# kokkos/kokkos-kernels

Measured on AMD Instinct MI355X. Metric: SpMV GFLOP/s (CSR, 27-pt 3-D FE Laplacian, fp64), higher is better.
Workload: dtype f64

## Files before the change

### kokkos-kernels_amd/csrc/kk_spmv_mv4.h

```cpp
#pragma once
#include "kk_spmv_plan.h"
#include <climits>

namespace kk {

constexpr int kMv4Threads = 512, kMv4RI = 32, kMv4RJ = 4, kMv4MaxL = 28;
__host__ __device__ constexpr int mv4_pitch(int ne, int vbytes) {
  return ((ne * vbytes) % 128 == 0) ? ne + 2 * (8 / vbytes) : ne;
}

struct Mv4Tab { int n; int e[kMv4MaxL]; };
constexpr int kMv4MaxG = 9;
struct Mv4Groups {
  int n, ng;
  int e[kMv4MaxG];
  int pres[kMv4MaxG];
  int perm[kMv4MaxL];
  int ent[kMv4MaxL];
};

}

struct kkamd_mv4_plan {
  int nx = 0, ny = 0, nz = 0, kc = 0, kc1 = 0, kc1_planes = 0;
  int64_t S1 = 0, S2 = 0, npi = 0, npj = 0, nchunk = 0, nchunk1 = 0, n_nc = 0;
  kk::Mv4Groups grp{};
  void* d_arow = nullptr;
  uint32_t* d_amask = nullptr;
  int32_t* d_nc = nullptr;
  size_t bytes = 0;
};

namespace kk {

template <class OffT, class AT>
__global__ __launch_bounds__(kBlock) void mv4_rows_kernel(int64_t n_list, const int32_t* __restrict__ list, const OffT* __restrict__ row_map,
                                                          const int32_t* __restrict__ entries, const AT* __restrict__ values,
                                                          const double* __restrict__ X, int64_t xs0, int64_t xs1, double* __restrict__ Y,
                                                          int64_t ys0, int64_t ys1, double alpha, double beta, int ncv) {
  int64_t idx = ((int64_t)blockIdx.x * kBlock + threadIdx.x) / 16;
  const int j  = threadIdx.x & 15;
  const int jc = j < ncv ? j : ncv - 1;
  const bool live = idx < n_list;
  if (!live) idx = n_list - 1;
  const int64_t r = list[idx];
  const int64_t b = (int64_t)row_map[r], e = (int64_t)row_map[r + 1];
  double acc = 0.0;
  for (int64_t a = b; a < e; a += 16) {
    const bool in = a + j < e;
    const int32_t my_col = in ? entries[a + j] : 0;
    const double my_val  = in ? (double)values[a + j] : 0.0;
    KK_UNROLL
    for (int q = 0; q < 16; ++q) {
      const int32_t col = __shfl(my_col, q, 16);
      const double v    = __shfl(my_val, q, 16);
      const double x    = X[(int64_t)col * xs0 + jc * xs1];
      acc = (a + q < e) ? acc + v * x : acc;
    }
  }
  if (!live || j >= ncv) return;
  double* yp = Y + r * ys0 + j * ys1;
  *yp = (beta == 0.0) ? alpha * acc : beta * (*yp) + alpha * acc;
}

template <class OffT, class AT, int NG, unsigned PRES, bool BETA0, int XM, bool PART = false>
__global__ __launch_bounds__(kMv4Threads, 1) void spmv_mv4_kernel(const OffT* __restrict__ arow, const uint32_t* __restrict__ amask, const AT* __restrict__ values, Mv4Groups G,
                                                                  const double* __restrict__ X0, int64_t xs0, int64_t xs1, double* __restrict__ Y0,
                                                                  int64_t ys0, int64_t ys1, double alpha, double beta, int y_vec_ok, int nx,
                                                                  int ny, int nz, int64_t S1, int64_t S2, int64_t npi, int64_t npj, int kc, int ncv_last, int ncb) {
  constexpr bool XROW = XM == 1;
  constexpr bool XT   = XM == 2;
  constexpr int RI = kMv4RI, RJ = kMv4RJ, W = RI + 2, SLABR = (RJ + 2) * W, SLABB = SLABR * 128, NT = kMv4Threads;
  constexpr int ROWS = NT / 8;
  constexpr int NP = SLABR * 8, NXP = (NP + NT - 1) / NT;
  constexpr int NPOS = 3 * NG + (NG & 1);
  constexpr int LP = mv4_pitch(NPOS, (int)sizeof(AT));
  constexpr int AV = (3 * NG + 7) / 8;
  using XV = kk_f64x2;
  using AV2 = typename vec2<AT>::type;
  KK_DYN_SMEM(char, smem);
  __shared__ int perm_s[kMv4MaxL];
  char* ring = smem;
  AT* abuf   = reinterpret_cast<AT*>(smem + 4 * (size_t)SLABB);
  const int t = threadIdx.x, rs = t >> 3, line = rs / RI, ii = rs % RI, c = t & 7;
  const int64_t bb = xcd_remap(blockIdx.x, gridDim.x);
  const int64_t b = ncb > 1 ? bb / ncb : bb;
  const int64_t cblk = ncb > 1 ? bb - b * ncb : 0;
  const double* __restrict__ X = X0 + cblk * 16 * xs1;
  double* __restrict__ Y = Y0 + cblk * 16 * ys1;
  const int ncv = (PART && cblk != ncb - 1) ? 16 : ncv_last;
  const int64_t npatch = npi * npj;
  const int64_t ch = b / npatch, p = b % npatch;
  const int i0 = (int)(p % npi) * RI, j0 = (int)(p / npi) * RJ;
  const int kbeg = (int)ch * kc, kend = (kbeg + kc < nz) ? kbeg + kc : nz;
  const int njj = (j0 + RJ <= ny) ? RJ : ny - j0;
  bool lane_ok[2];
  const OffT* wbase[2]; const uint32_t* mbase[2]; double* ybase[2];
  KK_UNROLL
  for (int u = 0; u < 2; ++u) {
    const int jj = 2 * line + u;
    lane_ok[u] = jj < njj && i0 + ii < nx;
    const int64_t r0 = lane_ok[u] ? (int64_t)(j0 + jj) * S1 + i0 + ii : 0;
    wbase[u] = arow + r0; mbase[u] = amask + r0;
    ybase[u] = Y + r0 * ys0 + (2 * c) * ys1;
  }
  const bool ycol0 = !PART || 2 * c < ncv, ycol1 = !PART || 2 * c + 1 < ncv;
  const double* xbase[NXP];
  unsigned xsec_none = 0;
  bool x_in[NXP];
  int x_dst[XT ? NXP : 1];
  unsigned x_live = 0;
  KK_UNROLL
  for (int it = 0; it < NXP; ++it) {
    int g = it * NT + t;
    int xr, part;
    if constexpr (!XT) { g = g < NP ? g : NP - 1; xr = g >> 3; part = g & 7; }
    else {
      part = g / SLABR; xr = g - part * SLABR;
      if (part > 7) { part = 7; xr = SLABR; }
      if (xr < SLABR) x_live |= 1u << it; else xr = SLABR - 1;
      x_dst[it] = (xr * 8 + (part ^ ((xr % W) & 7))) * 16;
    }
    const int jr = j0 - 1 + xr / W, ir = i0 - 1 + xr % W;
    x_in[it] = jr >= 0 && jr < ny && ir >= 0 && ir < nx;
    const int jq = jr < 0 ? 0 : (jr > ny - 1 ? ny - 1 : jr), iq = ir < 0 ? 0 : (ir > nx - 1 ? nx - 1 : ir);
    const int col0 = !PART ? 2 * part : (XROW ? (2 * part + 1 < ncv ? 2 * part : ncv - 2) : (2 * part < ncv ? 2 * part : ncv - 1));
    xbase[it] = X + ((int64_t)jq * S1 + iq) * xs0 + col0 * xs1;
    if (PART && !XROW && 2 * part + 1 >= ncv) xsec_none |= 1u << it;
  }
  auto plane_clamped = [&](int kp) -> int64_t { return kp < 0 ? 0 : (kp > nz - 1 ? nz - 1 : kp); };
  auto conforms = [&](int k, int u, OffT w) { return lane_ok[u] && k < kend && w >= 0; };
  auto load_words = [&](int kp, OffT (&w)[2], uint32_t (&mk)[2]) {
    const int64_t off = plane_clamped(kp) * S2;
    KK_UNROLL
    for (int u = 0; u < 2; ++u) { w[u] = wbase[u][off]; mk[u] = mbase[u][off]; }
  };
  auto load_slab = [&](int kp, XV (&rx)[NXP]) {
    const int64_t off = plane_clamped(kp) * S2 * xs0;
    KK_UNROLL
    for (int it = 0; it < NXP; ++it) {
      if constexpr (XROW) rx[it] = *reinterpret_cast<const XV*>(xbase[it] + off);
      else if constexpr (PART) { rx[it][0] = xbase[it][off]; rx[it][1] = xbase[it][off + (((xsec_none >> it) & 1u) ? 0 : xs1)]; }
      else { rx[it][0] = xbase[it][off]; rx[it][1] = xbase[it][off + xs1]; }
    }
  };
  auto zero_halo = [&](int kp) {
    if (kp > kend) return;
    char* dst = ring + (size_t)(kp & 3) * SLABB;
    const bool plane_in = kp >= 0 && kp < nz;
    const XV zero = {0.0, 0.0};
    KK_UNROLL
    for (int it = 0; it < NXP; ++it) {
      if constexpr (!XT) {
        const int g = it * NT + t;
        if (g < NP && !(plane_in && x_in[it])) *reinterpret_cast<XV*>(dst + (size_t)g * 16) = zero;
      } else {
        if (((x_live >> it) & 1u) && !(plane_in && x_in[it])) *reinterpret_cast<XV*>(dst + x_dst[it]) = zero;
      }
    }
  };
  auto store_slab = [&](int kp, const XV (&rx)[NXP]) {
    if (kp > kend || kp < 0 || kp >= nz) return;
    char* dst = ring + (size_t)(kp & 3) * SLABB;
    KK_UNROLL
    for (int it = 0; it < NXP; ++it) {
      if constexpr (!XT) {
        const int g = it * NT + t;
        if (g < NP && x_in[it]) *reinterpret_cast<XV*>(dst + (size_t)g * 16) = rx[it];
      } else {
        if (((x_live >> it) & 1u) && x_in[it]) *reinterpret_cast<XV*>(dst + x_dst[it]) = rx[it];
      }
    }
  };
  const uint32_t full = G.n >= 32 ? 0xffffffffu : ((1u << G.n) - 1u);
  KK_UNROLL
  for (int q = 0; q < kMv4MaxL; ++q) if (t == q) perm_s[q] = G.perm[q];
  __syncthreads();
  int qoff[AV], qpos[AV];
  KK_UNROLL
  for (int m = 0; m < AV; ++m) { qoff[m] = (c + 8 * m < G.n) ? c + 8 * m : G.n - 1; qpos[m] = perm_s[qoff[m]]; }
  auto load_values = [&](int k, const OffT (&w)[2], const uint32_t (&mk)[2], AT (&ra)[2][AV]) {
    KK_UNROLL
    for (int u = 0; u < 2; ++u) {
      const bool cf = conforms(k, u, w[u]);
      const AT* vb = values + (cf ? (int64_t)w[u] : 0);
      const bool part = cf && mk[u] != full;
      if (!__any(part)) {
        KK_UNROLL
        for (int m = 0; m < AV; ++m) ra[u][m] = vb[qoff[m]];
      } else {
        const uint32_t mask = cf ? mk[u] : 1u;
        KK_UNROLL
        for (int m = 0; m < AV; ++m) {
          const int q = c + 8 * m;
          ra[u][m] = vb[((mask >> q) & 1u) ? __popc(mask & ((1u << q) - 1u)) : 0];
        }
      }
    }
  };
  auto store_values = [&](int buf, const uint32_t (&mk)[2], const AT (&ra)[2][AV]) {
    KK_UNROLL
    for (int u = 0; u < 2; ++u) {
      AT* dst = abuf + ((size_t)(buf * 2 + u) * ROWS + rs) * LP;
      KK_UNROLL
      for (int m = 0; m < AV; ++m) { const int q = c + 8 * m; if (q < G.n) dst[qpos[m]] = ((mk[u] >> q) & 1u) ? ra[u][m] : AT(0); }
    }
  };
  auto y_ptr = [&](int k, int u) -> double* { return ybase[u] + (int64_t)k * S2 * ys0; };
  auto load_yold = [&](int k, const OffT (&w)[2], XV (&yo)[2]) {
    KK_UNROLL
    for (int u = 0; u < 2; ++u) {
      if (conforms(k, u, w[u])) {
        const double* yp = y_ptr(k, u);
        if constexpr (PART) { if (ycol1 && y_vec_ok) yo[u] = *reinterpret_cast<const XV*>(yp); else { if (ycol0) yo[u][0] = yp[0]; if (ycol1) yo[u][1] = yp[ys1]; } }
        else if (y_vec_ok) yo[u] = *reinterpret_cast<const XV*>(yp); else { yo[u][0] = yp[0]; yo[u][1] = yp[ys1]; }
      }
    }
  };

  OffT w_cur[2], w_nxt[2], w_stage[2][2];
  uint32_t m_cur[2], m_nxt[2], m_stage[2][2];
  AT ra[2][2][AV];
  XV rx[2][NXP];
  load_words(kbeg, w_cur, m_cur); load_words(kbeg + 1, w_nxt, m_nxt); load_words(kbeg + 2, w_stage[1], m_stage[1]);
  load_values(kbeg, w_cur, m_cur, ra[0]);
  {
    XV rt[NXP];
    load_slab(kbeg - 1, rx[0]); load_slab(kbeg, rx[1]); load_slab(kbeg + 1, rt);
    zero_halo(kbeg - 1); zero_halo(kbeg); zero_halo(kbeg + 1); zero_halo(kbeg + 2);
    store_slab(kbeg - 1, rx[0]); store_slab(kbeg, rx[1]); store_slab(kbeg + 1, rt);
  }
  store_values(0, m_cur, ra[0]);
  load_slab(kbeg + 2, rx[1]);
  load_values(kbeg + 1, w_nxt, m_nxt, ra[1]);
  __syncthreads();
  for (int kk = kbeg; kk < kend; kk += 2) {
    KK_UNROLL
    for (int P = 0; P < 2; ++P) {
      const int k = kk + P;
      if (k >= kend) break;
      load_words(k + 3, w_stage[P], m_stage[P]);
      load_slab(k + 3, rx[P]);
      load_values(k + 2, w_stage[1 - P], m_stage[1 - P], ra[P]);
      XV yold[2] = {{0.0, 0.0}, {0.0, 0.0}}, out[2] = {{0.0, 0.0}, {0.0, 0.0}};
      if constexpr (!BETA0) load_yold(k, w_cur, yold);
      if (conforms(k, 0, w_cur[0]) || conforms(k, 1, w_cur[1])) {
        const AT* av0 = abuf + ((size_t)(P * 2) * ROWS + rs) * LP;
        const AT* av1 = av0 + (size_t)ROWS * LP;
        const char* own = ring + (((2 * line) * W + ii + 1) << 7) + (XT ? 0 : c * 16);
        const char* own_d[3] = {own + ((c ^ (ii & 7)) << 4), own + ((c ^ ((ii + 1) & 7)) << 4), own + ((c ^ ((ii + 2) & 7)) << 4)};
        double a00 = 0.0, a01 = 0.0, a10 = 0.0, a11 = 0.0;
        KK_UNROLL
        for (int gp = 0; gp < (NG + 1) / 2; ++gp) {
          AV2 v0[3], v1[3];
          KK_UNROLL
          for (int i = 0; i < 3; ++i)
            if (6 * gp + 2 * i < NPOS) { v0[i] = *reinterpret_cast<const AV2*>(av0 + 6 * gp + 2 * i); v1[i] = *reinterpret_cast<const AV2*>(av1 + 6 * gp + 2 * i); }
          KK_UNROLL
          for (int gg = 0; gg < 2; ++gg) {
            const int g = 2 * gp + gg;
            if (g >= NG || (!PRES && g >= G.ng)) continue;
            const int e = G.e[g], pres = PRES ? (int)((PRES >> (3 * g)) & 7u) : G.pres[g];
            const int d_i = XT ? (((e >> 2) + W + 1) % W) : 0;
            const char* xb = (!XT ? own : (d_i == 0 ? own_d[0] : (d_i == 1 ? own_d[1] : own_d[2]))) + ((k + (e & 3) - 1) & 3) * SLABB + (e >> 2) * 128;
            XV x[4];
            KK_UNROLL
            for (int sl = 0; sl < 4; ++sl)
              if ((sl < 3 && ((pres >> sl) & 1)) || (sl > 0 && ((pres >> (sl - 1)) & 1))) x[sl] = *reinterpret_cast<const XV*>(xb + sl * (W * 128));
            KK_UNROLL
            for (int d = 0; d < 3; ++d) {
              if (!((pres >> d) & 1)) continue;
              const int idx = 3 * gg + d;
              const double va0 = (double)v0[idx >> 1][idx & 1], va1 = (double)v1[idx >> 1][idx & 1];
              a00 = __builtin_fma(va0, x[d][0], a00);     a01 = __builtin_fma(va0, x[d][1], a01);
              a10 = __builtin_fma(va1, x[d + 1][0], a10); a11 = __builtin_fma(va1, x[d + 1][1], a11);
            }
          }
        }
        out[0][0] = alpha * a00; out[0][1] = alpha * a01; out[1][0] = alpha * a10; out[1][1] = alpha * a11;
      }
      store_values(1 - P, m_nxt, ra[1 - P]);
      store_slab(k + 2, rx[1 - P]);
      KK_UNROLL
      for (int u = 0; u < 2; ++u) {
        if (conforms(k, u, w_cur[u])) {
          double* yp = y_ptr(k, u);
          if constexpr (!BETA0) { out[u][0] += beta * yold[u][0]; out[u][1] += beta * yold[u][1]; }
          if constexpr (PART) { if (ycol1 && y_vec_ok) *reinterpret_cast<XV*>(yp) = out[u]; else { if (ycol0) yp[0] = out[u][0]; if (ycol1) yp[ys1] = out[u][1]; } }
          else if (y_vec_ok) *reinterpret_cast<XV*>(yp) = out[u]; else { yp[0] = out[u][0]; yp[ys1] = out[u][1]; }
        }
      }
      __syncthreads();
      zero_halo(k + 3);
      KK_UNROLL
      for (int u = 0; u < 2; ++u) { w_cur[u] = w_nxt[u]; w_nxt[u] = w_stage[1 - P][u]; m_nxt[u] = m_stage[1 - P][u]; }
    }
  }
}

template <class OffT>
__global__ __launch_bounds__(kBlock) void mv4_verify_kernel(int64_t nrows, const OffT* __restrict__ row_map, const int32_t* __restrict__ entries,
                                                            Mv4Tab offs, Mv4Tab steps, int nx, int ny, int nz, OffT* __restrict__ arow,
                                                            uint32_t* __restrict__ amask, unsigned long long* __restrict__ count) {
  constexpr int CAP = kBlock * kMv4MaxL;
  __shared__ int s_ent[CAP];
  __shared__ long long s_off[kMv4MaxL];
  __shared__ int s_step[kMv4MaxL];
  if (threadIdx.x < kMv4MaxL) { s_off[threadIdx.x] = threadIdx.x < offs.n ? (long long)offs.e[threadIdx.x] : LLONG_MIN; s_step[threadIdx.x] = threadIdx.x < steps.n ? steps.e[threadIdx.x] : 0; }
  const int64_t r0 = (int64_t)blockIdx.x * kBlock, r = r0 + threadIdx.x;
  const int64_t rN = r0 + kBlock < nrows ? r0 + kBlock : nrows;
  const int64_t a0 = (int64_t)row_map[r0], a1 = (int64_t)row_map[rN];
  const bool staged = a1 - a0 <= CAP;
  if (staged) {
    for (int64_t p = threadIdx.x; p < a1 - a0; p += kBlock) s_ent[p] = entries[a0 + p];
  }
  __syncthreads();
  if (r >= nrows) return;
  const int64_t b = (int64_t)row_map[r], len = (int64_t)row_map[r + 1] - b;
  const int i = (int)(r % nx), j = (int)((r / nx) % ny), k = (int)(r / ((int64_t)nx * ny));
  auto inside = [&](int q) {
    const int s = s_step[q], kk = k + (s & 3) - 1, jj = j + ((s >> 2) & 3) - 1, ii = i + ((s >> 4) & 3) - 1;
    return kk >= 0 && kk < nz && jj >= 0 && jj < ny && ii >= 0 && ii < nx;
  };
  bool ok = len >= 1 && len <= offs.n;
  uint32_t mask = 0;
  int q = 0;
  for (int64_t a = 0; ok && a < len; ++a) {
    const int64_t d = (int64_t)(staged ? s_ent[b - a0 + a] : entries[b + a]) - r;
    while (q < offs.n && s_off[q] != d) ++q;
    ok = q < offs.n && inside(q);
    if (ok) mask |= 1u << q++;
  }
  for (int z = 0; ok && z < offs.n; ++z) ok = ((mask >> z) & 1u) || !inside(z);
  arow[r]  = ok ? (OffT)b : (OffT)-1;
  amask[r] = ok ? mask : 0u;
  if (!ok) atomicAdd(count, 1ull);
}
template <class OffT>
__global__ __launch_bounds__(kBlock) void mv4_list_kernel(int64_t nrows, const OffT* __restrict__ arow, int32_t* __restrict__ list,
                                                          unsigned long long* __restrict__ cursor) {
  const int64_t r = (int64_t)blockIdx.x * blockDim.x + threadIdx.x;
  if (r < nrows && arow[r] < 0) list[atomicAdd(cursor, 1ull)] = (int32_t)r;
}

template <class OffT>
int launch_mv4_verify(int64_t nrows, const OffT* row_map, const int32_t* entries, Mv4Tab offs, Mv4Tab steps, int nx, int ny, int nz, OffT* arow, uint32_t* amask,
                      unsigned long long* count, hipStream_t st)
#ifdef KK_MV4_INSTANTIATE
{
  KK_LAUNCH((mv4_verify_kernel<OffT>), (unsigned)ceil_div(nrows, kBlock), kBlock, 0, st, nrows, row_map, entries, offs, steps, nx, ny, nz, arow, amask, count);
  return KKAMD_OK;
}
#else
;
#endif
template <class OffT>
int launch_mv4_list(int64_t nrows, const OffT* arow, int32_t* list, unsigned long long* count, hipStream_t st)
#ifdef KK_MV4_INSTANTIATE
{
  KK_LAUNCH((mv4_list_kernel<OffT>), (unsigned)ceil_div(nrows, kBlock), kBlock, 0, st, nrows, arow, list, count);
  return KKAMD_OK;
}
#else
;
#endif
#ifndef KK_MV4_INSTANTIATE
extern template int launch_mv4_verify<int32_t>(int64_t, const int32_t*, const int32_t*, Mv4Tab, Mv4Tab, int, int, int, int32_t*, uint32_t*, unsigned long long*, hipStream_t);
extern template int launch_mv4_verify<int64_t>(int64_t, const int64_t*, const int32_t*, Mv4Tab, Mv4Tab, int, int, int, int64_t*, uint32_t*, unsigned long long*, hipStream_t);
extern template int launch_mv4_list<int32_t>(int64_t, const int32_t*, int32_t*, unsigned long long*, hipStream_t);
extern template int launch_mv4_list<int64_t>(int64_t, const int64_t*, int32_t*, unsigned long long*, hipStream_t);
#endif

template <class OffT, class AT, int NE, unsigned FL>
int launch_mv4_stencil(const kkamd_mv4_plan* m, const kkamd_crs_t* A, const double* X, int64_t xs0, int64_t xs1, double* Y, int64_t ys0, int64_t ys1,
                       double alpha, double beta, hipStream_t st, int ncv, int ncb, bool xrow, bool xcol)
#ifdef KK_MV4_INSTANTIATE
{
  const size_t slabs = 4 * (size_t)((kMv4RJ + 2) * (kMv4RI + 2) * 128), rows = kMv4Threads / 8;
  const int yv = (ys1 == 1 && (ys0 % 2 == 0) && ((uintptr_t)Y % 16 == 0)) ? 1 : 0;
  const bool part = ncv < 16;
#ifndef KK_EMU
#define KK_MV4_ATTR(B0, XR, PT) KK_HIP(hipFuncSetAttribute(reinterpret_cast<const void*>(&spmv_mv4_kernel<OffT, AT, NE, FL, B0, XR, PT>), hipFuncAttributeMaxDynamicSharedMemorySize, (int)lds))
#else
#define KK_MV4_ATTR(B0, XR, PT) (void)0
#endif
#define KK_MV4B(B0, XR, PT)                                                                                                        \
  do {                                                                                                                          \
    const size_t lds = slabs + 4 * rows * mv4_pitch(3 * NE + (NE & 1), (int)sizeof(AT)) * sizeof(AT);                            \
    KK_MV4_ATTR(B0, XR, PT);                                                                                                      \
    KK_LAUNCH((spmv_mv4_kernel<OffT, AT, NE, FL, B0, XR, PT>), (unsigned)(m->npi * m->npj * m->nchunk * ncb), kMv4Threads, lds, st,  \
              (const OffT*)m->d_arow, (const uint32_t*)m->d_amask, (const AT*)A->d_values, m->grp, X, xs0, xs1, Y, ys0, ys1, alpha, \
              beta, yv, m->nx, m->ny, m->nz, m->S1, m->S2, m->npi, m->npj, m->kc, ncv, ncb);                                     \
  } while (0)
  if (part) {
    if (beta == 0.0) { if (xrow && ncv % 2 == 0) KK_MV4B(true, 1, true); else if (xcol) KK_MV4B(true, 2, true); else KK_MV4B(true, 0, true); }
    else { if (xrow && ncv % 2 == 0) KK_MV4B(false, 1, true); else if (xcol) KK_MV4B(false, 2, true); else KK_MV4B(false, 0, true); }
  }
  else if (beta == 0.0) { if (xrow) KK_MV4B(true, 1, false); else if (xcol) KK_MV4B(true, 2, false); else KK_MV4B(true, 0, false); }
  else { if (xrow) KK_MV4B(false, 1, false); else if (xcol) KK_MV4B(false, 2, false); else KK_MV4B(false, 0, false); }
#undef KK_MV4B
#undef KK_MV4_ATTR
  KK_LAUNCH_CHECK();
  return KKAMD_OK;
}
#else
;
#endif

template <class OffT, class AT>
int launch_mv4_rows(const kkamd_mv4_plan* m, const kkamd_crs_t* A, const double* X, int64_t xs0, int64_t xs1, double* Y, int64_t ys0, int64_t ys1,
                    double alpha, double beta, hipStream_t st, int ncv, int ncb)
#ifdef KK_MV4_INSTANTIATE
{
  for (int q = 0; q < ncb; ++q) {
    const double* Xq = X + (int64_t)q * 16 * xs1; double* Yq = Y + (int64_t)q * 16 * ys1;
    const int ncv_q = q == ncb - 1 ? ncv : 16;
    KK_LAUNCH((mv4_rows_kernel<OffT, AT>), (unsigned)ceil_div(m->n_nc * 16, (int64_t)kBlock), kBlock, 0, st, m->n_nc, (const int32_t*)m->d_nc,
              (const OffT*)A->d_row_map, (const int32_t*)A->d_entries, (const AT*)A->d_values, Xq, xs0, xs1, Yq, ys0, ys1, alpha, beta, ncv_q);
    KK_LAUNCH_CHECK();
  }
  return KKAMD_OK;
}
#else
;
#endif

constexpr unsigned kMv4Pat27 = 0x7FFFFFFu;
constexpr unsigned kMv4Pat7  = 2u | 2u << 3 | 7u << 6 | 2u << 9 | 2u << 12;
#define KK_MV4_FOR_ALL(F) F(int32_t, double) F(int32_t, float) F(int64_t, double) F(int64_t, float)
#define KK_MV4_DECL(OT, AT_)                                                                                                                                \
  extern template int launch_mv4_stencil<OT, AT_, 9, kMv4Pat27>(const kkamd_mv4_plan*, const kkamd_crs_t*, const double*, int64_t, int64_t, double*, int64_t, int64_t, double, double, hipStream_t, int, int, bool, bool); \
  extern template int launch_mv4_stencil<OT, AT_, 5, kMv4Pat7>(const kkamd_mv4_plan*, const kkamd_crs_t*, const double*, int64_t, int64_t, double*, int64_t, int64_t, double, double, hipStream_t, int, int, bool, bool);  \
  extern template int launch_mv4_stencil<OT, AT_, 5, 0u>(const kkamd_mv4_plan*, const kkamd_crs_t*, const double*, int64_t, int64_t, double*, int64_t, int64_t, double, double, hipStream_t, int, int, bool, bool);        \
  extern template int launch_mv4_stencil<OT, AT_, 9, 0u>(const kkamd_mv4_plan*, const kkamd_crs_t*, const double*, int64_t, int64_t, double*, int64_t, int64_t, double, double, hipStream_t, int, int, bool, bool);        \
  extern template int launch_mv4_rows<OT, AT_>(const kkamd_mv4_plan*, const kkamd_crs_t*, const double*, int64_t, int64_t, double*, int64_t, int64_t, double, double, hipStream_t, int, int);
#ifndef KK_MV4_INSTANTIATE
KK_MV4_FOR_ALL(KK_MV4_DECL)
#endif
#undef KK_MV4_DECL

template <class OffT, class AT>
inline int launch_mv4(const kkamd_spmv_plan* plan, const kkamd_crs_t* A, const double* X, int64_t xs0, int64_t xs1, double* Y, int64_t ys0, int64_t ys1,
                      double alpha, double beta, hipStream_t st, int ncv = 16, int ncb = 1) {
  const kkamd_mv4_plan* m = plan->mv4;
  const bool xrow = xs1 == 1 && (xs0 % 2 == 0) && ((uintptr_t)X % 16 == 0);
  const bool xcol = xs0 == 1 && plan->tune.mv4_xcol;
  unsigned pat = 0;
  for (int g = 0; g < m->grp.ng; ++g) pat |= (unsigned)m->grp.pres[g] << (3 * g);
  int rc;
  if (m->grp.ng == 9 && pat == kMv4Pat27) rc = launch_mv4_stencil<OffT, AT, 9, kMv4Pat27>(m, A, X, xs0, xs1, Y, ys0, ys1, alpha, beta, st, ncv, ncb, xrow, xcol);
  else if (m->grp.ng == 5 && pat == kMv4Pat7) rc = launch_mv4_stencil<OffT, AT, 5, kMv4Pat7>(m, A, X, xs0, xs1, Y, ys0, ys1, alpha, beta, st, ncv, ncb, xrow, xcol);
  else if (m->grp.ng <= 5) rc = launch_mv4_stencil<OffT, AT, 5, 0u>(m, A, X, xs0, xs1, Y, ys0, ys1, alpha, beta, st, ncv, ncb, xrow, xcol);
  else rc = launch_mv4_stencil<OffT, AT, 9, 0u>(m, A, X, xs0, xs1, Y, ys0, ys1, alpha, beta, st, ncv, ncb, xrow, xcol);
  if (rc) return rc;
  if (m->n_nc > 0) return launch_mv4_rows<OffT, AT>(m, A, X, xs0, xs1, Y, ys0, ys1, alpha, beta, st, ncv, ncb);
  return KKAMD_OK;
}

}
```

Baseline: 1376.

## Remap XT stencil threads to i-pairs and reuse x loads across groups

In the column-major X (XT) path of the mv4 stencil kernel, each thread now handles two adjacent i positions in the same j line instead of two j lines. This lets x vectors loaded from the shared-memory ring be reused across stencil groups with a compile-time pattern, through a cached xc array and a constexpr need-mask. The LDS swizzle layout is changed to match, and Y loads and stores pair adjacent rows into 16-byte vector accesses when parity allows. Pattern specialisations now also check the group offsets before being used. The cost is more register pressure and more complex indexing.

```diff
diff --git a/kokkos-kernels_amd/csrc/kk_spmv_mv4.h b/kokkos-kernels_amd/csrc/kk_spmv_mv4.h
--- a/kokkos-kernels_amd/csrc/kk_spmv_mv4.h
+++ b/kokkos-kernels_amd/csrc/kk_spmv_mv4.h
@@ -18,6 +18,21 @@
   int perm[kMv4MaxL];
   int ent[kMv4MaxL];
 };
+constexpr unsigned kMv4Pat27 = 0x7FFFFFFu;
+constexpr unsigned kMv4Pat7  = 2u | 2u << 3 | 7u << 6 | 2u << 9 | 2u << 12;
+__host__ __device__ constexpr int mv4_pat_e(unsigned pat, int g) {
+  return pat == kMv4Pat27 ? ((g / 3) | ((g % 3 - 1) * 4)) : (g == 0 ? 0 : g == 1 ? (1 | (-1 * 4)) : g == 2 ? 1 : g == 3 ? (1 | 4) : 2);
+}
+__host__ __device__ constexpr int mv4_pat_groups(unsigned pat) { return pat == kMv4Pat27 ? 9 : 5; }
+__host__ __device__ constexpr bool mv4_pat_need(unsigned pat, int dk1, int l, int tt) {
+  for (int g = 0; g < mv4_pat_groups(pat); ++g) {
+    const int e = mv4_pat_e(pat, g), di = e >> 2;
+    if ((e & 3) == dk1 && ((pat >> (3 * g + l)) & 1u) && (tt == di + 1 || tt == di + 2)) return true;
+  }
+  return false;
+}
+__host__ __device__ constexpr int mv4_xt_pos(int iw) { return iw ^ ((iw >> 1) & 1); }
+__host__ __device__ constexpr int mv4_xt_slot(int iw) { return ((iw & 3) << 1) | ((iw >> 2) & 1); }
 
 }
 
@@ -83,6 +98,7 @@
   char* ring = smem;
   AT* abuf   = reinterpret_cast<AT*>(smem + 4 * (size_t)SLABB);
   const int t = threadIdx.x, rs = t >> 3, line = rs / RI, ii = rs % RI, c = t & 7;
+  const int pj = rs / (RI / 2), ip = rs % (RI / 2);
   const int64_t bb = xcd_remap(blockIdx.x, gridDim.x);
   const int64_t b = ncb > 1 ? bb / ncb : bb;
   const int64_t cblk = ncb > 1 ? bb - b * ncb : 0;
@@ -98,9 +114,9 @@
   const OffT* wbase[2]; const uint32_t* mbase[2]; double* ybase[2];
   KK_UNROLL
   for (int u = 0; u < 2; ++u) {
-    const int jj = 2 * line + u;
-    lane_ok[u] = jj < njj && i0 + ii < nx;
-    const int64_t r0 = lane_ok[u] ? (int64_t)(j0 + jj) * S1 + i0 + ii : 0;
+    const int jj = XT ? pj : 2 * line + u, il = XT ? 2 * ip + u : ii;
+    lane_ok[u] = jj < njj && i0 + il < nx;
+    const int64_t r0 = lane_ok[u] ? (int64_t)(j0 + jj) * S1 + i0 + il : 0;
     wbase[u] = arow + r0; mbase[u] = amask + r0;
     ybase[u] = Y + r0 * ys0 + (2 * c) * ys1;
   }
@@ -119,7 +135,7 @@
       part = g / SLABR; xr = g - part * SLABR;
       if (part > 7) { part = 7; xr = SLABR; }
       if (xr < SLABR) x_live |= 1u << it; else xr = SLABR - 1;
-      x_dst[it] = (xr * 8 + (part ^ ((xr % W) & 7))) * 16;
+      x_dst[it] = (((xr / W) * W + mv4_xt_pos(xr % W)) * 8 + (part ^ mv4_xt_slot(xr % W))) * 16;
     }
     const int jr = j0 - 1 + xr / W, ir = i0 - 1 + xr % W;
     x_in[it] = jr >= 0 && jr < ny && ir >= 0 && ir < nx;
@@ -207,13 +223,26 @@
     }
   };
   auto y_ptr = [&](int k, int u) -> double* { return ybase[u] + (int64_t)k * S2 * ys0; };
+  const int y_par = (int)((reinterpret_cast<uintptr_t>(ybase[0]) >> 3) & 1);
+  auto y_pair = [&](int k, int cc, bool cf0, bool cf1) {
+    return ys0 == 1 && cf0 && cf1 && (cc == 0 ? ycol0 : ycol1) && ((y_par ^ (k & (int)S2) ^ (cc & (int)ys1)) & 1) == 0;
+  };
   auto load_yold = [&](int k, const OffT (&w)[2], XV (&yo)[2]) {
-    KK_UNROLL
-    for (int u = 0; u < 2; ++u) {
-      if (conforms(k, u, w[u])) {
-        const double* yp = y_ptr(k, u);
-        if constexpr (PART) { if (ycol1 && y_vec_ok) yo[u] = *reinterpret_cast<const XV*>(yp); else { if (ycol0) yo[u][0] = yp[0]; if (ycol1) yo[u][1] = yp[ys1]; } }
-        else if (y_vec_ok) yo[u] = *reinterpret_cast<const XV*>(yp); else { yo[u][0] = yp[0]; yo[u][1] = yp[ys1]; }
+    if constexpr (XT) {
+      const bool cf0 = conforms(k, 0, w[0]), cf1 = conforms(k, 1, w[1]);
+      KK_UNROLL
+      for (int cc = 0; cc < 2; ++cc) {
+        if (y_pair(k, cc, cf0, cf1)) yo[cc] = *reinterpret_cast<const XV*>(y_ptr(k, 0) + cc * ys1);
+        else if (cc == 0 ? ycol0 : ycol1) { if (cf0) yo[cc][0] = y_ptr(k, 0)[cc * ys1]; if (cf1) yo[cc][1] = y_ptr(k, 1)[cc * ys1]; }
+      }
+    } else {
+      KK_UNROLL
+      for (int u = 0; u < 2; ++u) {
+        if (conforms(k, u, w[u])) {
+          const double* yp = y_ptr(k, u);
+          if constexpr (PART) { if (ycol1 && y_vec_ok) yo[u] = *reinterpret_cast<const XV*>(yp); else { if (ycol0) yo[u][0] = yp[0]; if (ycol1) yo[u][1] = yp[ys1]; } }
+          else if (y_vec_ok) yo[u] = *reinterpret_cast<const XV*>(yp); else { yo[u][0] = yp[0]; yo[u][1] = yp[ys1]; }
+        }
       }
     }
   };
@@ -247,9 +276,14 @@
       if (conforms(k, 0, w_cur[0]) || conforms(k, 1, w_cur[1])) {
         const AT* av0 = abuf + ((size_t)(P * 2) * ROWS + rs) * LP;
         const AT* av1 = av0 + (size_t)ROWS * LP;
-        const char* own = ring + (((2 * line) * W + ii + 1) << 7) + (XT ? 0 : c * 16);
-        const char* own_d[3] = {own + ((c ^ (ii & 7)) << 4), own + ((c ^ ((ii + 1) & 7)) << 4), own + ((c ^ ((ii + 2) & 7)) << 4)};
+        const char* own = ring + ((XT ? pj * W : (2 * line) * W + ii + 1) << 7) + (XT ? 0 : c * 16);
+        const char* own_t[XT ? 4 : 1];
+        if constexpr (XT) {
+          KK_UNROLL
+          for (int tt = 0; tt < 4; ++tt) own_t[tt] = own + (mv4_xt_pos(2 * ip + tt) << 7) + ((c ^ mv4_xt_slot(2 * ip + tt)) << 4);
+        }
         double a00 = 0.0, a01 = 0.0, a10 = 0.0, a11 = 0.0;
+        XV xc[XT && PRES ? 3 : 1][4];
         KK_UNROLL
         for (int gp = 0; gp < (NG + 1) / 2; ++gp) {
           AV2 v0[3], v1[3];
@@ -260,34 +294,96 @@
           for (int gg = 0; gg < 2; ++gg) {
             const int g = 2 * gp + gg;
             if (g >= NG || (!PRES && g >= G.ng)) continue;
-            const int e = G.e[g], pres = PRES ? (int)((PRES >> (3 * g)) & 7u) : G.pres[g];
-            const int d_i = XT ? (((e >> 2) + W + 1) % W) : 0;
-            const char* xb = (!XT ? own : (d_i == 0 ? own_d[0] : (d_i == 1 ? own_d[1] : own_d[2]))) + ((k + (e & 3) - 1) & 3) * SLABB + (e >> 2) * 128;
-            XV x[4];
-            KK_UNROLL
-            for (int sl = 0; sl < 4; ++sl)
-              if ((sl < 3 && ((pres >> sl) & 1)) || (sl > 0 && ((pres >> (sl - 1)) & 1))) x[sl] = *reinterpret_cast<const XV*>(xb + sl * (W * 128));
-            KK_UNROLL
-            for (int d = 0; d < 3; ++d) {
-              if (!((pres >> d) & 1)) continue;
-              const int idx = 3 * gg + d;
-              const double va0 = (double)v0[idx >> 1][idx & 1], va1 = (double)v1[idx >> 1][idx & 1];
-              a00 = __builtin_fma(va0, x[d][0], a00);     a01 = __builtin_fma(va0, x[d][1], a01);
-              a10 = __builtin_fma(va1, x[d + 1][0], a10); a11 = __builtin_fma(va1, x[d + 1][1], a11);
+            const int pres = PRES ? (int)((PRES >> (3 * g)) & 7u) : G.pres[g];
+            if constexpr (!XT) {
+              const int e = G.e[g];
+              const char* xb = own + ((k + (e & 3) - 1) & 3) * SLABB + (e >> 2) * 128;
+              XV x[4];
+              KK_UNROLL
+              for (int sl = 0; sl < 4; ++sl)
+                if ((sl < 3 && ((pres >> sl) & 1)) || (sl > 0 && ((pres >> (sl - 1)) & 1))) x[sl] = *reinterpret_cast<const XV*>(xb + sl * (W * 128));
+              KK_UNROLL
+              for (int d = 0; d < 3; ++d) {
+                if (!((pres >> d) & 1)) continue;
+                const int idx = 3 * gg + d;
+                const double va0 = (double)v0[idx >> 1][idx & 1], va1 = (double)v1[idx >> 1][idx & 1];
+                a00 = __builtin_fma(va0, x[d][0], a00);     a01 = __builtin_fma(va0, x[d][1], a01);
+                a10 = __builtin_fma(va1, x[d + 1][0], a10); a11 = __builtin_fma(va1, x[d + 1][1], a11);
+              }
+            } else if constexpr (PRES != 0) {
+              const int e = mv4_pat_e(PRES, g), di = e >> 2;
+              if (g == 0 || (mv4_pat_e(PRES, g - 1) & 3) != (e & 3)) {
+                const int slab = ((k + (e & 3) - 1) & 3) * SLABB;
+                KK_UNROLL
+                for (int l = 0; l < 3; ++l) {
+                  KK_UNROLL
+                  for (int tt = 0; tt < 4; ++tt)
+                    if (mv4_pat_need(PRES, e & 3, l, tt)) xc[l][tt] = *reinterpret_cast<const XV*>(own_t[tt] + slab + l * (W * 128));
+                }
+              }
+              KK_UNROLL
+              for (int d = 0; d < 3; ++d) {
+                if (!((pres >> d) & 1)) continue;
+                const int idx = 3 * gg + d;
+                const double va0 = (double)v0[idx >> 1][idx & 1], va1 = (double)v1[idx >> 1][idx & 1];
+                a00 = __builtin_fma(va0, xc[d][di + 1][0], a00); a01 = __builtin_fma(va0, xc[d][di + 1][1], a01);
+                a10 = __builtin_fma(va1, xc[d][di + 2][0], a10); a11 = __builtin_fma(va1, xc[d][di + 2][1], a11);
+              }
+            } else {
+              const int e = G.e[g], di = e >> 2;
+              const int slab = ((k + (e & 3) - 1) & 3) * SLABB;
+              const char* xb0 = (di < 0 ? own_t[0] : (di == 0 ? own_t[1] : own_t[2])) + slab;
+              const char* xb1 = (di < 0 ? own_t[1] : (di == 0 ? own_t[2] : own_t[3])) + slab;
+              XV x0[3], x1[3];
+              KK_UNROLL
+              for (int l = 0; l < 3; ++l)
+                if ((pres >> l) & 1) { x0[l] = *reinterpret_cast<const XV*>(xb0 + l * (W * 128)); x1[l] = *reinterpret_cast<const XV*>(xb1 + l * (W * 128)); }
+              KK_UNROLL
+              for (int d = 0; d < 3; ++d) {
+                if (!((pres >> d) & 1)) continue;
+                const int idx = 3 * gg + d;
+                const double va0 = (double)v0[idx >> 1][idx & 1], va1 = (double)v1[idx >> 1][idx & 1];
+                a00 = __builtin_fma(va0, x0[d][0], a00); a01 = __builtin_fma(va0, x0[d][1], a01);
+                a10 = __builtin_fma(va1, x1[d][0], a10); a11 = __builtin_fma(va1, x1[d][1], a11);
+              }
             }
           }
         }
-        out[0][0] = alpha * a00; out[0][1] = alpha * a01; out[1][0] = alpha * a10; out[1][1] = alpha * a11;
+        if constexpr (XT) { out[0][0] = alpha * a00; out[1][0] = alpha * a01; out[0][1] = alpha * a10; out[1][1] = alpha * a11; }
+        else { out[0][0] = alpha * a00; out[0][1] = alpha * a01; out[1][0] = alpha * a10; out[1][1] = alpha * a11; }
       }
       store_values(1 - P, m_nxt, ra[1 - P]);
       store_slab(k + 2, rx[1 - P]);
-      KK_UNROLL
-      for (int u = 0; u < 2; ++u) {
-        if (conforms(k, u, w_cur[u])) {
-          double* yp = y_ptr(k, u);
-          if constexpr (!BETA0) { out[u][0] += beta * yold[u][0]; out[u][1] += beta * yold[u][1]; }
-          if constexpr (PART) { if (ycol1 && y_vec_ok) *reinterpret_cast<XV*>(yp) = out[u]; else { if (ycol0) yp[0] = out[u][0]; if (ycol1) yp[ys1] = out[u][1]; } }
-          else if (y_vec_ok) *reinterpret_cast<XV*>(yp) = out[u]; else { yp[0] = out[u][0]; yp[ys1] = out[u][1]; }
+      if constexpr (XT) {
+        const bool cf0 = conforms(k, 0, w_cur[0]), cf1 = conforms(k, 1, w_cur[1]);
+        if constexpr (!BETA0) {
+          KK_UNROLL
+          for (int cc = 0; cc < 2; ++cc) { out[cc][0] += beta * yold[cc][0]; out[cc][1] += beta * yold[cc][1]; }
+        }
+        if (y_vec_ok) {
+          KK_UNROLL
+          for (int u = 0; u < 2; ++u) {
+            if (!(u == 0 ? cf0 : cf1)) continue;
+            double* yp = y_ptr(k, u);
+            const XV o = {out[0][u], out[1][u]};
+            if (ycol1) *reinterpret_cast<XV*>(yp) = o; else if (ycol0) yp[0] = o[0];
+          }
+        } else {
+          KK_UNROLL
+          for (int cc = 0; cc < 2; ++cc) {
+            if (y_pair(k, cc, cf0, cf1)) *reinterpret_cast<XV*>(y_ptr(k, 0) + cc * ys1) = out[cc];
+            else if (cc == 0 ? ycol0 : ycol1) { if (cf0) y_ptr(k, 0)[cc * ys1] = out[cc][0]; if (cf1) y_ptr(k, 1)[cc * ys1] = out[cc][1]; }
+          }
+        }
+      } else {
+        KK_UNROLL
+        for (int u = 0; u < 2; ++u) {
+          if (conforms(k, u, w_cur[u])) {
+            double* yp = y_ptr(k, u);
+            if constexpr (!BETA0) { out[u][0] += beta * yold[u][0]; out[u][1] += beta * yold[u][1]; }
+            if constexpr (PART) { if (ycol1 && y_vec_ok) *reinterpret_cast<XV*>(yp) = out[u]; else { if (ycol0) yp[0] = out[u][0]; if (ycol1) yp[ys1] = out[u][1]; } }
+            else if (y_vec_ok) *reinterpret_cast<XV*>(yp) = out[u]; else { yp[0] = out[u][0]; yp[ys1] = out[u][1]; }
+          }
         }
       }
       __syncthreads();
@@ -425,8 +521,6 @@
 ;
 #endif
 
-constexpr unsigned kMv4Pat27 = 0x7FFFFFFu;
-constexpr unsigned kMv4Pat7  = 2u | 2u << 3 | 7u << 6 | 2u << 9 | 2u << 12;
 #define KK_MV4_FOR_ALL(F) F(int32_t, double) F(int32_t, float) F(int64_t, double) F(int64_t, float)
 #define KK_MV4_DECL(OT, AT_)                                                                                                                                \
   extern template int launch_mv4_stencil<OT, AT_, 9, kMv4Pat27>(const kkamd_mv4_plan*, const kkamd_crs_t*, const double*, int64_t, int64_t, double*, int64_t, int64_t, double, double, hipStream_t, int, int, bool, bool); \
@@ -447,9 +541,13 @@
   const bool xcol = xs0 == 1 && plan->tune.mv4_xcol;
   unsigned pat = 0;
   for (int g = 0; g < m->grp.ng; ++g) pat |= (unsigned)m->grp.pres[g] << (3 * g);
+  auto groups_of = [&](unsigned p) {
+    for (int g = 0; g < m->grp.ng; ++g) if (m->grp.e[g] != mv4_pat_e(p, g)) return false;
+    return true;
+  };
   int rc;
-  if (m->grp.ng == 9 && pat == kMv4Pat27) rc = launch_mv4_stencil<OffT, AT, 9, kMv4Pat27>(m, A, X, xs0, xs1, Y, ys0, ys1, alpha, beta, st, ncv, ncb, xrow, xcol);
-  else if (m->grp.ng == 5 && pat == kMv4Pat7) rc = launch_mv4_stencil<OffT, AT, 5, kMv4Pat7>(m, A, X, xs0, xs1, Y, ys0, ys1, alpha, beta, st, ncv, ncb, xrow, xcol);
+  if (m->grp.ng == 9 && pat == kMv4Pat27 && groups_of(kMv4Pat27)) rc = launch_mv4_stencil<OffT, AT, 9, kMv4Pat27>(m, A, X, xs0, xs1, Y, ys0, ys1, alpha, beta, st, ncv, ncb, xrow, xcol);
+  else if (m->grp.ng == 5 && pat == kMv4Pat7 && groups_of(kMv4Pat7)) rc = launch_mv4_stencil<OffT, AT, 5, kMv4Pat7>(m, A, X, xs0, xs1, Y, ys0, ys1, alpha, beta, st, ncv, ncb, xrow, xcol);
   else if (m->grp.ng <= 5) rc = launch_mv4_stencil<OffT, AT, 5, 0u>(m, A, X, xs0, xs1, Y, ys0, ys1, alpha, beta, st, ncv, ncb, xrow, xcol);
   else rc = launch_mv4_stencil<OffT, AT, 9, 0u>(m, A, X, xs0, xs1, Y, ys0, ys1, alpha, beta, st, ncv, ncb, xrow, xcol);
   if (rc) return rc;
```

Measured after the change: 1356. -1.4%, worse.
